# JohnGoertz/Gumbi

Hardware: AMD Instinct MI355X
Metric: fit+predict achieved GFLOP/s (fp64 exact GP: one MAP objective + gradient evaluation at the model's starting hyper-parameters + grid prediction) (higher is better)
Workload: dtype f64; 1 GPU; synthetic N=50k d=8 Matern-5/2 ARD fp64, M=10^4 grid; N=50000, d=8, kernel=Matern52, M=10000, parallelism=1 GPU, warmup_step=the same step (untimed)

## Files before the change

gumbi_amd/csrc/engine.hip:

```cpp
#include <hip/hip_runtime.h>

#include <algorithm>
#include <cmath>
#include <cstdarg>
#include <cstdio>
#include <cstdlib>
#include <cstring>
#include <string>
#include <functional>
#include <unordered_map>
#include <mutex>
#include <memory>
#include <vector>

#include "../../include/gumbi_hip.h"
#include "device_buffers.hpp"
#include "workspaces.hpp"
#include "term_walk.hpp"
#include "factor_state.hpp"
#include "eval_plan.hpp"
#include "covariance.hpp"
#include "gemm_f64.hpp"
#include "gemm_splitk.hpp"
#include "gradient.hpp"
// ... 84 lines not shown
  std::string err;

  int64_t N = 0, Np = 0, Nr = 0, ld = 0;
  int32_t D = 0;
  DevPool pool;
  DevBuf<double> dX, dy, dA;
  DevBuf<double> dDinv16;

  gmb_kernel_spec spec{};
  bool have_spec = false, have_theta = false;
  std::vector<double> theta;
  int nc_pad = 1;
  int periodic = 0;
  double periods[8] = {};
  PreparedPoints pts;
  DevBuf<double> dtabs, dnoise;
  struct Term {
    PrepArgs pa;
    CovParams cp;
    double eta;
    int n_tab_acc;
  };
  std::vector<Term> terms;
  std::vector<double> htabs;
  std::vector<double> hnoise;

  DevBuf<double> dscal;
  int32_t* dinfo = nullptr;
  DevBuf<double> dv;
  FactorState fs;
  DevBuf<double> dDiagSave;
  DevBuf<double> dsk;
  int64_t notpd = -1;
  double logdet = 0.0, vnorm2 = 0.0;

  PredictWorkspace pw;
  int predict_form = -1;
  GemmFormWorkspace pw2;
  JointState jt;
  DevBuf<double> dpart;
  PredictGradWorkspace pg;
  DevBuf<double> pg_part;
  DevBuf<double> dalpha_bs;
  DevBuf<double> vg_grad;
  TermsWorkspace tg;
  GroupWorkspace ga;
  DevBuf<double> ga_part;
  SlopeWorkspace slope;
  DevBuf<int64_t> ga_idx;
  DesignWorkspace dz;

  DevBuf<double> dW;
  DevBuf<double> dalpha;
  double* dgpart = nullptr;
  DevBuf<double> dgred;
  DevBuf<double> dgbig;

  struct InvLevelPlan {
    int variant[2] = {0, 0};
    int grid_x[2] = {0, 0};
    int count = 0;
    int64_t off[2] = {0, 0};
    int64_t toff = 0;
    int tr_rows = 0, tr_cols = 0;
    double flops[2] = {0.0, 0.0};
  };
  std::vector<InvLevelPlan> inv_plan;
  DevBuf<GemmArgs> dplan_gemm;
  DevBuf<TransposeJob> dplan_tr;
  int64_t plan_N = -1, plan_ld = -1, plan_Np = -1;
  const double* plan_W = nullptr;
  const double* plan_A = nullptr;
  bool batch_inverse = true;
  bool lpt_order = true;
  long long lpt_max_tiles = 16384;
  int cov_strip = 0;
  int tile_strip = 8;

  bool profiling = false;
  gmb_timings tm{};
  std::vector<EventPair> evs;
  bool naive_leaf = false;
  bool gemm_dma = true;
  bool small_tiles = true;
  int gemm_variant = 0;
  long long wg_slots = 512;
  bool force_variant = false;

  hipStream_t aux[3] = {nullptr, nullptr, nullptr};
  int chol_scheme = -1;
  DevBuf<uint32_t> dct;
  DevBuf<unsigned long long> dct_trace;
  bool ct_trace = false;
  CholResult chol;
  int ct_lose = 0;
  struct HostLanding {
    double scal[2];
    int32_t info;
    uint32_t abort;
    double gacc[GACC_DOUBLES];
  };
  HostLanding* hl = nullptr;
  HostLanding* hl_dev = nullptr;
  hipEvent_t fe[4] = {nullptr, nullptr, nullptr, nullptr};
  int inline_prep_max_rows = 4096;
  int grad_scheme = -1;
  int et_lag = -1;
  DevBuf<uint32_t> det_tasks;
  int et_key[5] = {-1, -1, -1, -1, -1};
  int et_pairs = -1;
  int et_pairs_min_blocks = 72;
  int et_ntasks = 0;
  DevBuf<double> dUdiag;
  DevBuf<double> dApart;
  int et_min_blocks = 1;
  int panel_tiles_w = 16;
  bool panel_tiles_veto = false;
  int tiles_min_blocks = 6, tiles_max_blocks = 224;
  int tiles_trsm_min_blocks = 16;
  int masked_max_blocks = 128;
  std::vector<hipEvent_t> sync_pool;
  size_t sync_next = 0;
  bool lookahead = true;
  bool par_inverse = true;
  bool aux_shared = false;
  bool aux_borrowed = false;
  int part_cus = 0;
  DevBuf<double> dsend, drecv;
  DevBuf<double> dsend2, drecv2;
  int panel_blocks = 8;
  bool panel_auto = true;
  int dist_mode = 0;
  DevBuf<double> dAown;
  int64_t ld_own = 0;
  int own_world = -1, own_rank = -1;
  DevBuf<double> dPanel;
  std::function<int(double*, int64_t, int)> solve_hook;
  DevBuf<double> dstat;
  uint64_t coll_count = 0, coll_hash = 0;
  std::vector<hipEvent_t> time_pool;
  size_t time_next = 0;
};

namespace {

int fail(gmb_engine* e, int code, const char* fmt, ...) {
  char buf[512];
  va_list ap;
  va_start(ap, fmt);
  vsnprintf(buf, sizeof buf, fmt, ap);
  va_end(ap);
  if (e) e->err = buf;
  return code;
}

#define HIP_TRY(e, call)                                                              \
  do {                                                                                \
    hipError_t _s = (call);                                                           \
    if (_s != hipSuccess)                                                             \
      return fail(e, GMB_EHIP, "%s failed: %s (%s:%d)", #call, hipGetErrorString(_s), \
                  __FILE__, __LINE__);                                                \
  } while (0)

int alloc_refused(void* owner, size_t bytes, const char* why) {
  return fail(static_cast<gmb_engine*>(owner), GMB_ENOMEM, "hipMalloc of %lld bytes failed: %s", (long long)bytes, why);
}
// ... 186 lines not shown
  if (g_in.mt <= 0 || g_in.nt <= 0 || g_in.k <= 0) return GMB_OK;
  GemmArgs g = g_in;
  if (g.nblk_stride < 1) g.nblk_stride = 1;
  const long long nact = gemm_nact128(g);
  const bool in_place = (const double*)g.C == g.B;
  int variant = e->gemm_variant;
  {
    static const double rate[4] = {73.0, 63.0, 65.0, 60.0};
    static const int per128[4] = {1, 4, 2, 4};
    const double slots = (double)e->wg_slots;
    auto score = [&](int v) {
      const double t = (double)(nact * per128[v]);
      const double rounds = std::max(1.0, t / slots + 0.5);
      return rate[v] * per128[v] / rounds;
    };
    if (in_place) {
      if (g.mt != 1) return fail(e, GMB_EINVAL, "internal: in-place GEMM needs m == 128");
      variant = 0;
      if (score(2) > score(variant)) variant = 2;
      if (score(3) > score(variant)) variant = 3;
      if (pin && pin->variant >= 0) {
        if (pin->variant != 0 && pin->variant != 2 && pin->variant != 3) return fail(e, GMB_EINVAL, "gemm pin: the in-place form runs on the 128-row tiles (variants 0, 2, 3)");
        variant = pin->variant;
      }
    } else if (pin && pin->variant >= 0) {
      if (pin->variant > 3) return fail(e, GMB_EINVAL, "gemm pin: variant %d", pin->variant);
      variant = pin->variant;
    } else if (!e->force_variant) {
      variant = 0;
      if (e->small_tiles) {
        if (score(2) > score(variant)) variant = 2;
        if (score(1) > score(variant)) variant = 1;
      }
    }
  }
#ifdef GMB_TUNING
  if (e->force_variant && e->gemm_variant == 4 && !in_place) variant = (g_in.mt % 2 == 0) ? 4 : 0;
#endif
  static const int BMs[5] = {128, 64, 128, 128, 256}, BNs[5] = {128, 64, 64, 32, 128};
  const int bm = BMs[variant], bn = BNs[variant];
  g.mt = g_in.mt * TILE / bm;
  g.nt = g_in.nt * TILE / bn;
  g.order = 0;
  if (e->lpt_order && nact <= e->lpt_max_tiles && g.nblk_stride == 1 && g.tri_off >= 0 && !g.klo_m && (g.klo_n != 0) != (g.khi_n != 0))
    g.order = g.klo_n ? 1 : 2;
  if (pin && pin->order >= 0) {
    const bool lpt_ok = g.nblk_stride == 1 && g.tri_off >= 0 && !g.klo_m && (g.klo_n != 0) != (g.khi_n != 0);
    if (pin->order > 2 || (pin->order != 0 && (!lpt_ok || pin->order != (g.klo_n ? 1 : 2))))
      return fail(e, GMB_EINVAL, "gemm pin: order %d is not one launch_gemm chooses for this product", pin->order);
    g.order = pin->order;
  }
  g.strip = (g.order == 0 && e->tile_strip > 0 && g.mt >= 2 && !in_place && !g.klo_m) ? e->tile_strip : 0;
  if (pin && pin->strip >= 0) {
    if (pin->strip > 255 || (pin->strip > 0 && !(g.order == 0 && g.mt >= 2 && !in_place && !g.klo_m)))
      return fail(e, GMB_EINVAL, "gemm pin: strip %d is not one launch_gemm chooses for this product", pin->strip);
    g.strip = pin->strip;
  }
  bool pfc = g.beta != 0.0 && g.k <= 1024 && !in_place;
  bool dma = e->gemm_dma && variant == 0 && !in_place;
  if (pin && pin->pfc >= 0) {
    if (pin->pfc > 1 || (pin->pfc == 1 && (g.beta == 0.0 || in_place || variant == 0)))
      return fail(e, GMB_EINVAL, "gemm pin: C prefetch needs beta != 0, an out-of-place product and a small tile");
    pfc = pin->pfc == 1;
  }
  if (pin && pin->staging >= 0) {
    if (pin->staging > 1 || (pin->staging == 1 && (variant != 0 || in_place)))
      return fail(e, GMB_EINVAL, "gemm pin: LDS-DMA staging exists for the out-of-place 128 x 128 tile only");
    dma = pin->staging == 1;
  }
  double flops = 0.0;
  const int nblocks = gemm_schedule(g, bm, bn, &flops);
  if (nblocks <= 0) return GMB_OK;
  const bool bulk_update = ev_kind == EV_CHOL_UPDATE && variant == 0 && !in_place;
  const int was_update = ev_kind == EV_CHOL_UPDATE ? (1 << 16) : 0;
  if (ev_kind == EV_CHOL_UPDATE && !bulk_update) ev_kind = EV_CHOL_PANEL_GEMM;
  ev_begin(e, s, ev_kind, flops, g_in.mt, g_in.nt, g.k,
           g.tri | (g.klo_n << 3) | (g.khi_n << 4) | (g.klo_m << 5) | (variant << 8) | was_update);
  const dim3 grid(nblocks);
  if (pin && pin->launched)
    *pin->launched = variant | (dma ? 4 : 0) | (variant != 0 && pfc ? 8 : 0) | (in_place ? 16 : 0) | (g.order << 5) | ((g.strip & 0xff) << 8) |
                     (std::min(nblocks, 0x7fff) << 16);
  switch (variant) {
    case 0:
      if (dma && bulk_update) hipLaunchKernelGGL(gemm_f64_dma_chol_update_kernel, grid, dim3(256), 0, s, g);
      else if (dma) hipLaunchKernelGGL(gemm_f64_dma_kernel, grid, dim3(256), 0, s, g);
      else hipLaunchKernelGGL((gemm_f64_kernel<2, 2, 4, 4, 2>), grid, dim3(256), 0, s, g);
      break;
#ifdef GMB_TUNING
    case 4: hipLaunchKernelGGL((gemm_f64_kernel<4, 2, 4, 4, 1>), grid, dim3(512), 0, s, g); break;
#endif
    case 1:
      if (pfc) hipLaunchKernelGGL((gemm_f64_kernel<2, 2, 2, 2, 2, true>), grid, dim3(256), 0, s, g);
      else hipLaunchKernelGGL((gemm_f64_kernel<2, 2, 2, 2, 2>), grid, dim3(256), 0, s, g);
      break;
    case 2:
      if (pfc) hipLaunchKernelGGL((gemm_f64_kernel<2, 2, 4, 2, 2, true>), grid, dim3(256), 0, s, g);
      else hipLaunchKernelGGL((gemm_f64_kernel<2, 2, 4, 2, 2>), grid, dim3(256), 0, s, g);
      break;
    default:
      if (pfc) hipLaunchKernelGGL((gemm_f64_kernel<2, 2, 4, 1, 2, true>), grid, dim3(256), 0, s, g);
      else hipLaunchKernelGGL((gemm_f64_kernel<2, 2, 4, 1, 2>), grid, dim3(256), 0, s, g);
      break;
  }
  ev_end(e);
  HIP_TRY(e, hipGetLastError());
  return GMB_OK;
}

int launch_trsm_strip(gmb_engine* e, hipStream_t s, double* B, int64_t ldb, int64_t nrows, const double* L, int64_t ldl,
                      const double* dinv16, int nvalid, EvKind ev_kind) {
  if (nrows <= 0) return GMB_OK;
  TrsmArgs t;
  t.B = B;
  t.ldb = ldb;
  t.nrows = nrows;
  t.L = L;
  t.ldl = ldl;
  t.dinv16 = dinv16;
  t.nvalid = nvalid;
  ev_begin(e, s, ev_kind, (double)nrows * TILE * TILE);
  hipLaunchKernelGGL(trsm_strip_kernel, dim3((unsigned)((nrows / 16 + 3) / 4)), dim3(256), 0, s, t);
  ev_end(e);
  HIP_TRY(e, hipGetLastError());
  return GMB_OK;
}

int launch_leaf(gmb_engine* e, hipStream_t s, const LeafArgs& a) {
  ev_begin(e, s, EV_LEAF, 0.0);
  if (e->naive_leaf)
    hipLaunchKernelGGL(potrf_leaf_naive_kernel, dim3(1), dim3(256), 0, s, a);
  else
    hipLaunchKernelGGL(potrf_leaf_kernel, dim3(1), dim3(512), 0, s, a);
  ev_end(e);
  HIP_TRY(e, hipGetLastError());
  return GMB_OK;
}

long long cov_grid_blocks(int ti, int tj, int strip, int tri_grid, int row_first, int row_stride) {
  const int S = strip < 1 ? 1 : strip;
  const long long nst = (tj + S - 1) / S;
  if (row_stride > 0) return row_first < ti ? ((ti - 1 - row_first) / row_stride + 1) * nst : 0;
  if (tri_grid) return cov_tri_blocks_before(ti, tj, S);
  return (long long)ti * nst;
}

template <int KIND>
int launch_cov_nc(gmb_engine* e, const CovTileArgs& a, int nc) {
  const long long nb = cov_grid_blocks(a.ti, a.tj, a.strip, a.tri_grid, a.row_first, a.row_stride) * (a.gsplit > 1 ? a.gsplit : 1);
  if (nb <= 0) return GMB_OK;
  const dim3 grid((unsigned)nb), block(256);
  switch (nc) {
    case 1: hipLaunchKernelGGL((cov_tile_kernel<KIND, 1>), grid, block, 0, e->stream, a); break;
    case 2: hipLaunchKernelGGL((cov_tile_kernel<KIND, 2>), grid, block, 0, e->stream, a); break;
    case 4: hipLaunchKernelGGL((cov_tile_kernel<KIND, 4>), grid, block, 0, e->stream, a); break;
    case 8: hipLaunchKernelGGL((cov_tile_kernel<KIND, 8>), grid, block, 0, e->stream, a); break;
    default: hipLaunchKernelGGL((cov_tile_kernel<KIND, 16>), grid, block, 0, e->stream, a); break;
  }
  HIP_TRY(e, hipGetLastError());
  return GMB_OK;
}

int launch_cov(gmb_engine* e, const CovTileArgs& a_in) {
  if (a_in.ti <= 0 || a_in.tj <= 0) return GMB_OK;
  CovTileArgs a = a_in;
  const double tiles = (double)a.ti * a.tj * (a.lower_only ? 0.5 : 1.0) / (a.row_stride > 0 ? a.row_stride : 1);
  a.stream_stores = tiles * TILE * TILE * 8.0 >= 1073741824.0 / (a.row_stride > 0 ? a.row_stride : 1);
  a.strip = e->cov_strip > 0 ? e->cov_strip : (tiles >= 32768.0 ? 4 : tiles >= 12288.0 ? 2 : 1);
// ... 1309 lines not shown
      }
    }
  if (k != (int)e->theta.size()) return fail(e, GMB_EINVAL, "internal: gradient packing mismatch");
  return GMB_OK;
}

inline bool chol_scheme_valid(int s) { return s == -1 || s == 0 || s == 2 || s == 3 || s == 4; }

int require_ready(gmb_engine* e, bool need_factor) {
  if (!e) return GMB_EINVAL;
  if (e->N <= 0) return fail(e, GMB_EINVAL, "gmb_set_data has not been called");
  if (!e->have_spec) return fail(e, GMB_EINVAL, "gmb_set_kernel has not been called");
  if (!e->have_theta) return fail(e, GMB_EINVAL, "gmb_set_theta has not been called");
  if (need_factor && !e->fs.valid())
    return fail(e, GMB_EINVAL, "no valid factorisation: call gmb_factorize first");
  return GMB_OK;
}

int require_full_factor(gmb_engine* e, const char* what) {
  if (e->fs.capacity() || !e->dA || e->dA.cap <= 0)
    return fail(e, GMB_EINVAL, "%s needs the complete factor on this device, but the resident factorisation is a capacity-mode one "
                               "(gmb_dist_set_mode(e, 1): no rank holds the factor) -- use the gmb_dist_* calls, or gmb_factorize first", what);
  return GMB_OK;
}

int require_capacity_factor(gmb_engine* e, const char* what) {
  if (!e->fs.capacity() || !e->dAown)
    return fail(e, GMB_EINVAL, "%s in capacity mode needs a factorisation made by gmb_dist_factorize in capacity mode; the resident "
                               "one was made by %s", what, e->fs.single() ? "gmb_factorize / gmb_evaluate" : "the replicated multi-GPU driver");
  return GMB_OK;
}

}

namespace {

hipStream_t shared_masked_stream(int device, int part_cus, int* ncu_out) {
  static std::mutex mu;
  static hipStream_t streams[64] = {};
  static int ncus[64] = {};
  std::lock_guard<std::mutex> lock(mu);
  hipStream_t& st = streams[device & 63];
  if (!st) {
    hipDeviceProp_t prop;
    if (hipGetDeviceProperties(&prop, device) != hipSuccess) return nullptr;
    const int ncu = prop.multiProcessorCount;
    std::vector<uint32_t> mask((ncu + 31) / 32, 0u);
    for (int i = part_cus; i < ncu; ++i) mask[i / 32] |= 1u << (i % 32);
    if (hipExtStreamCreateWithCUMask(&st, (uint32_t)mask.size(), mask.data()) != hipSuccess) {
      st = nullptr;
      (void)hipGetLastError();
      return nullptr;
    }
    ncus[device & 63] = ncu;
  }
  if (ncu_out) *ncu_out = ncus[device & 63];
  return st;
}

int gmb_create_impl(gmb_engine** out, int32_t device, void* stream, const gmb_engine* peer = nullptr) {
  if (!out) return GMB_EINVAL;
  *out = nullptr;
  int n = gmb_device_count();
  if (n < 0) return GMB_ENODEVICE;
  if (device < 0 || device >= n) return GMB_EINVAL;
  if (hipSetDevice(device) != hipSuccess) return GMB_EHIP;
  gmb_engine* e = new gmb_engine();
  e->device = device;
  if (stream) {
    e->stream = (hipStream_t)stream;
  } else {
    if (hipStreamCreateWithFlags(&e->stream, hipStreamNonBlocking) != hipSuccess) {
      delete e;
      return GMB_EHIP;
    }
    e->own_stream = true;
  }
  auto flag = [](const char* name, bool dflt) {
    const char* v = getenv(name);
    return v && v[0] ? v[0] != '0' : dflt;
  };
  e->naive_leaf = flag("GMB_LEAF_NAIVE", false);
  e->gemm_dma = flag("GMB_GEMM_DMA", true);
  const char* cs = getenv("GMB_CHOL_SCHEME");
  if (cs && cs[0]) {
    const int v = atoi(cs);
    if (chol_scheme_valid(v)) e->chol_scheme = v;
    else fprintf(stderr, "[gumbi_hip] GMB_CHOL_SCHEME=%s ignored: valid schemes are -1 (by size), 0, 2, 3, 4\n", cs);
  }
  int part = 32;
#ifdef GMB_TUNING
  e->small_tiles = flag("GMB_SMALL_TILES", true);
  const char* gv = getenv("GMB_GEMM_VARIANT");
  if (gv && gv[0] >= '0' && gv[0] <= '4') {
    e->gemm_variant = gv[0] - '0';
    e->force_variant = true;
  }
  e->lookahead = flag("GMB_LOOKAHEAD", true);
  e->lpt_order = flag("GMB_LPT_ORDER", true);
  if (const char* lm = getenv("GMB_LPT_MAX_TILES")) e->lpt_max_tiles = atoll(lm);
  const char* ts = getenv("GMB_TILE_STRIP");
  if (ts) e->tile_strip = std::max(0, atoi(ts));
  const char* cst = getenv("GMB_COV_STRIP");
  if (cst) e->cov_strip = std::max(0, std::min(64, atoi(cst)));
  e->batch_inverse = flag("GMB_BATCH_INVERSE", true);
  e->par_inverse = flag("GMB_PAR_INVERSE", true);
  const char* pb = getenv("GMB_PANEL_BLOCKS");
  if (pb && atoi(pb) > 0) {
    e->panel_blocks = atoi(pb);
    e->panel_auto = false;
  }
  const char* mb = getenv("GMB_MASKED_MAX_BLOCKS");
  if (mb) e->masked_max_blocks = atoi(mb);
  if (const char* pw = getenv("GMB_PANEL_TILES_W")) e->panel_tiles_w = std::max(0, std::min(64, atoi(pw)));
  const char* pc = getenv("GMB_PART_CUS");
  if (pc) part = atoi(pc);
#endif
  int prio_lo = 0, prio_hi = 0;
  (void)hipDeviceGetStreamPriorityRange(&prio_lo, &prio_hi);
  for (int a = 0; a < 3 && peer; ++a) {
    e->aux[a] = peer->aux[a];
    e->aux_borrowed = true;
    e->aux_shared = peer->aux_shared;
    e->part_cus = peer->part_cus;
  }
  for (int a = 0; a < 3 && !peer; ++a) {
    hipError_t st2 = hipSuccess;
    int ncu = 0;
    hipStream_t masked = (a == 2 && part > 0) ? shared_masked_stream(device, part, &ncu) : nullptr;
    if (masked) {
      e->aux[a] = masked;
      e->aux_shared = true;
      e->part_cus = part;
    } else {
      st2 = hipStreamCreateWithPriority(&e->aux[a], hipStreamNonBlocking, a == 2 ? prio_lo : prio_hi);
    }
    if (st2 != hipSuccess) {
      gmb_destroy(e);
      return GMB_EHIP;
    }
  }
  hipDeviceProp_t prop;
  if (hipGetDeviceProperties(&prop, device) == hipSuccess) e->wg_slots = 2LL * prop.multiProcessorCount;
  e->pool.owner = e;
  e->pool.refused = alloc_refused;
  if (e->dscal.renew(e->pool, SCAL_DOUBLES, false) || e->dstat.renew(e->pool, (DIST_HEADER + DIST_MAX_PAYLOAD) * (1 + DIST_MAX_WORLD), false)) {
    gmb_destroy(e);
    return GMB_ENOMEM;
  }
  e->dinfo = reinterpret_cast<int32_t*>(e->dscal + SCAL_INFO_AT);
  e->dgpart = e->dscal + SCAL_GACC_AT;
  *out = e;
  return GMB_OK;
}

}

extern "C" {

int gmb_abi_version(void) { return GMB_ABI_VERSION; }

int gmb_device_count(void) {
  int n = 0;
  hipError_t s = hipGetDeviceCount(&n);
  if (s != hipSuccess || n <= 0) return GMB_ENODEVICE;
  return n;
// ... 2577 lines not shown
  if (!out || ldo < e->Nr) return fail(e, GMB_EINVAL, "gmb_blk_covariance: out is null or ldo < %lld", (long long)e->Nr);
  if ((((uintptr_t)out) | (uintptr_t)(ldo * (int64_t)sizeof(double))) & 15u)
    return fail(e, GMB_EINVAL, "gmb_blk_covariance: out must be 16-byte aligned and ldo even (16-byte stores)");
  HIP_TRY(e, hipSetDevice(e->device));
  if ((rc = build_sigma(e, out, ldo))) return rc;
  HIP_TRY(e, hipStreamSynchronize(e->stream));
  return GMB_OK;
}

int gmb_blk_potrf(gmb_engine* e, double* Akk, int64_t lda, int32_t nvalid, double* dinv16,
                  double* logdet_accum, int32_t* info) {
  if (!e || !Akk || nvalid < 1 || nvalid > TILE || lda < TILE) return fail(e, GMB_EINVAL, "bad potrf block");
  HIP_TRY(e, hipSetDevice(e->device));
  LeafArgs a{};
  a.A = Akk;
  a.lda = lda;
  a.nvalid = nvalid;
  a.dinv16 = dinv16;
  a.logdet = logdet_accum;
  a.info = info ? info : e->dinfo;
  a.row0 = 0;
#ifdef GMB_TUNING
  a.dbg = getenv("GMB_LEAF_DBG") ? logdet_accum + 1 : nullptr;
#else
  a.dbg = nullptr;
#endif
  return launch_leaf(e, e->stream, a);
}

int gmb_blk_invert(gmb_engine* e, const double* Lkk, int64_t lda, int32_t nvalid, const double* dinv16,
                   double* invLkk) {
  if (!e || !Lkk || !dinv16 || !invLkk || nvalid < 1 || nvalid > TILE || lda < TILE)
    return fail(e, GMB_EINVAL, "bad invert block");
  HIP_TRY(e, hipSetDevice(e->device));
  InvArgs ia{};
  ia.L = Lkk;
  ia.lda = lda;
  ia.blk_stride = 0;
  ia.dinv16 = dinv16;
  ia.invL = invLkk;
  ia.n = nvalid;
  hipLaunchKernelGGL(leaf_invert_kernel, dim3(1), dim3(256), 0, e->stream, ia);
  HIP_TRY(e, hipGetLastError());
  return GMB_OK;
}

int gmb_blk_trsm(gmb_engine* e, double* B, int64_t ldb, int64_t nrows, const double* Lkk, int64_t ldl,
                 const double* dinv16, int32_t nvalid) {
  if (!e || !B || !Lkk || !dinv16 || nrows < 0 || nrows % 16 || ldb < nrows || ldl < TILE || nvalid < 1 ||
      nvalid > TILE)
    return fail(e, GMB_EINVAL, "bad trsm arguments (rows must be a multiple of 16)");
  HIP_TRY(e, hipSetDevice(e->device));
  return launch_trsm_strip(e, e->stream, B, ldb, nrows, Lkk, ldl, dinv16, nvalid, EV_CHOL_STRIP);
}

int gmb_blk_gemm_nt(gmb_engine* e, double* C, int64_t ldc, const double* A, int64_t lda, const double* B,
                    int64_t ldb, int64_t m, int64_t n, int64_t k, double alpha, double beta, int32_t tri,
                    int64_t tri_shift) {
  if (!e || !C || !A || !B) return fail(e, GMB_EINVAL, "null gemm operand");
  if (m % TILE || n % TILE || k % KT || m < 0 || n < 0 || k < 0)
    return fail(e, GMB_EINVAL, "gemm sizes must be multiples of 128 (m, n) and 16 (k)");
  HIP_TRY(e, hipSetDevice(e->device));
  GemmArgs g{};
  g.C = C;
  g.ldc = ldc;
  g.A = A;
  g.lda = lda;
  g.B = B;
  g.ldb = ldb;
  g.mt = (int)(m / TILE);
  g.nt = (int)(n / TILE);
  g.k = (int)k;
  g.alpha = alpha;
  g.beta = beta;
  g.tri = tri;
  g.tri_off = (int)(tri_shift * TILE);
  return launch_gemm(e, e->stream, g, EV_CHOL_PANEL_GEMM);
}

int gmb_blk_gemm_ex(gmb_engine* e, double* C, const double* A, const double* B, const gmb_gemm_desc* d, int32_t* launched) {
  if (launched) *launched = 0;
  if (!e) return GMB_EINVAL;
  if (!C || !A || !B || !d) return fail(e, GMB_EINVAL, "null gemm operand");
  if (d->m % TILE || d->n % TILE || d->k % KT || d->m < 0 || d->n < 0 || d->k < 0 || d->m > (1 << 24) || d->n > (1 << 24) || d->k > (1 << 24))
    return fail(e, GMB_EINVAL, "gemm sizes must be multiples of 128 (m, n) and 16 (k)");
  if (((uintptr_t)A | (uintptr_t)B | (uintptr_t)(d->lda * 8) | (uintptr_t)(d->ldb * 8)) & 15u)
    return fail(e, GMB_EINVAL, "gmb_blk_gemm_ex: A and B must be 16-byte aligned, lda and ldb even");
  if (d->nblk_stride < 0 || d->cblk_stride < 0 || d->krow_stride < 0 || d->nblk_stride > 4096 || d->cblk_stride > 4096 || d->krow_stride > 4096 ||
      (d->klo_m | d->klo_n | d->khi_n | d->tri) < 0 || (d->klo_m | d->klo_n | d->khi_n | d->tri) > 1)
    return fail(e, GMB_EINVAL, "gmb_blk_gemm_ex: strides must be >= 0, tri / klo_m / klo_n / khi_n 0 or 1");
  if (d->tri_off % 32 || d->krow_off % TILE) return fail(e, GMB_EINVAL, "gmb_blk_gemm_ex: tri_off must be a multiple of 32, krow_off of 128");
  const int64_t bs = d->nblk_stride < 1 ? 1 : d->nblk_stride, cs = d->cblk_stride > 0 ? d->cblk_stride : bs;
  const int64_t brows = d->n ? ((d->n / TILE - 1) * bs + 1) * TILE : 0, crows = d->n ? ((d->n / TILE - 1) * cs + 1) * TILE : 0;
  if (d->lda < d->m || d->ldb < brows || d->ldc < crows) return fail(e, GMB_EINVAL, "gmb_blk_gemm_ex: a leading dimension is smaller than its operand");
  if ((const double*)C == B && d->ldc != d->ldb) return fail(e, GMB_EINVAL, "gmb_blk_gemm_ex: in place needs ldc == ldb");
  if (d->variant < -1 || d->staging < -1 || d->pfc < -1 || d->order < -1 || d->strip < -1) return fail(e, GMB_EINVAL, "gmb_blk_gemm_ex: a pin below -1");
  HIP_TRY(e, hipSetDevice(e->device));
  GemmArgs g{};
  g.C = C;
  g.ldc = d->ldc;
  g.A = A;
  g.lda = d->lda;
  g.B = B;
  g.ldb = d->ldb;
  g.mt = (int)(d->m / TILE);
  g.nt = (int)(d->n / TILE);
  g.k = (int)d->k;
  g.alpha = d->alpha;
  g.beta = d->beta;
  g.tri = d->tri;
  g.tri_off = d->tri_off;
  g.nblk_stride = d->nblk_stride;
  g.cblk_stride = d->cblk_stride;
  g.klo_m = d->klo_m;
  g.klo_n = d->klo_n;
  g.khi_n = d->khi_n;
  g.krow_off = d->krow_off;
  g.krow_stride = d->krow_stride;
  GemmPin pin;
  pin.variant = d->variant;
  pin.staging = d->staging;
  pin.pfc = d->pfc;
  pin.order = d->order;
  pin.strip = d->strip;
  pin.launched = launched;
  return launch_gemm(e, e->stream, g, EV_CHOL_PANEL_GEMM, &pin);
}

int gmb_blk_gemm_splitk(gmb_engine* e, double* C, int64_t ldc, const double* A, int64_t lda, const double* B, int64_t ldb, int64_t m,
                        int64_t n, int64_t k, double alpha, double beta, int32_t tri, int32_t slices, int32_t* slices_used) {
  if (slices_used) *slices_used = 0;
  if (!e) return GMB_EINVAL;
  if (!C || !A || !B) return fail(e, GMB_EINVAL, "null gemm operand");
  if (m % TILE || n % TILE || k % KT || m <= 0 || n <= 0 || k <= 0 || m > (1 << 24) || n > (1 << 24) || k > (1 << 24))
    return fail(e, GMB_EINVAL, "split-k gemm sizes must be positive multiples of 128 (m, n) and 16 (k)");
  if (((uintptr_t)A | (uintptr_t)B | (uintptr_t)(lda * 8) | (uintptr_t)(ldb * 8)) & 15u)
    return fail(e, GMB_EINVAL, "gmb_blk_gemm_splitk: A and B must be 16-byte aligned, lda and ldb even");
  if (lda < m || ldb < n || ldc < n) return fail(e, GMB_EINVAL, "gmb_blk_gemm_splitk: a leading dimension is smaller than its operand");
  if (tri < 0 || tri > 1) return fail(e, GMB_EINVAL, "gmb_blk_gemm_splitk: tri must be 0 or 1");
  if (slices != -1 && slices < 1) return fail(e, GMB_EINVAL, "gmb_blk_gemm_splitk: slices must be -1 (by the rule) or >= 1");
  HIP_TRY(e, hipSetDevice(e->device));
  SplitKArgs a{};
  a.C = C;
  a.ldc = ldc;
  a.A = A;
  a.lda = lda;
  a.B = B;
  a.ldb = ldb;
  a.mt = (int)(m / TILE);
  a.nt = (int)(n / TILE);
  a.k = (int)k;
  a.alpha = alpha;
  a.beta = beta;
  a.tri = tri;
  return launch_gemm_splitk(e, e->stream, a, slices, slices_used);
}

int gmb_append(gmb_engine* e, const double* Xnew, int64_t K, int64_t ldx, const double* ynew, int32_t memspace) {
  int rc = resize_ready(e, "gmb_append");
  if (rc) return rc;
  if (!Xnew || !ynew || K < 0 || ldx < e->D) return fail(e, GMB_EINVAL, "gmb_append: bad Xnew/K/ldx/ynew");
  if (K == 0) return GMB_OK;
  return resize_n(e, e->N + K, Xnew, K, ldx, ynew, memspace, "gmb_append");
}

int64_t gmb_num_obs(const gmb_engine* e) { return e ? e->N : (int64_t)GMB_EINVAL; }

int gmb_truncate(gmb_engine* e, int64_t n_keep) {
// ... 52 lines not shown
```

gumbi_amd/csrc/gemm_f64.hpp:

```cpp
#pragma once
#include <hip/hip_runtime.h>
#include <algorithm>
#include <stdint.h>

namespace gmb {

typedef double d4 __attribute__((ext_vector_type(4)));
typedef double d2 __attribute__((ext_vector_type(2)));

constexpr int TILE = 128;
constexpr int KT = 16;
constexpr int PITCH = TILE + 16;

struct GemmArgs {
  double* C;
  int64_t ldc;
  const double* A;
  int64_t lda;
  const double* B;
  int64_t ldb;
  int32_t mt, nt;
  int32_t k;
  double alpha, beta;
  int32_t tri;
  int32_t tri_off;
  int32_t nblk_stride;
  int32_t cblk_stride;
  int32_t klo_m, klo_n, khi_n;
  int32_t krow_off;
  int32_t krow_stride;
  int32_t xstart[9];
  int32_t order;
  int32_t strip;
  int32_t xs_t0[8], xs_base[8];
};

__host__ __device__ __forceinline__ int xcd_remap(int bid, int nwg) {
  const int q = nwg >> 3, r = nwg & 7;
  const int xcd = bid & 7, idx = bid >> 3;
  const int base = (xcd < r) ? xcd * (q + 1) : r * (q + 1) + (xcd - r) * q;
  return base + idx;
}

__host__ __device__ __forceinline__ int64_t gemm_noff(int tn, int bn, int stride) {
  const int64_t e = (int64_t)tn * bn;
  return (e >> 7) * stride * 128 + (e & 127);
}
__host__ __device__ __forceinline__ int gemm_first_tn(int64_t T, int bn, int stride) {
  if (T <= 0) return 0;
  const int per = 128 / bn;
  if (T < 0x7fffffff) {
    const uint32_t S = (uint32_t)stride * 128u, t = (uint32_t)T;
    const uint32_t q = t / S, r = t - q * S;
    if (r == 0) return (int)(q * per);
    if (r > (uint32_t)(128 - bn)) return (int)((q + 1) * per);
    return (int)(q * per + (r + bn - 1) / (uint32_t)bn);
  }
  const int64_t S = (int64_t)stride * 128;
  const int64_t q = T / S, r = T % S;
  if (r == 0) return (int)(q * per);
  if (r > 128 - bn) return (int)((q + 1) * per);
  return (int)(q * per + (r + bn - 1) / bn);
}

__host__ __device__ inline bool gemm_decode_tile(const GemmArgs& g, const int BM, const int BN, const int vbid, int& tm,
                                                 int& tn) {
  const int xcd = vbid & 7;
  int ci = g.xstart[xcd] + (vbid >> 3);
  if (g.order == 0 && g.strip > 0) {
    if (ci >= g.xstart[xcd + 1]) return false;
    auto first_of = [&](int t) {
      if (!g.tri) return 0;
      const int f = gemm_first_tn((int64_t)t * BM - g.tri_off - (BN - 1), BN, g.nblk_stride);
      return f > g.nt ? g.nt : f;
    };
    int t0 = g.xs_t0[xcd];
    ci -= g.xs_base[xcd];
    for (;;) {
      const int t1 = t0 + g.strip < g.mt ? t0 + g.strip : g.mt;
      int cnt = 0;
      for (int t = t0; t < t1; ++t) cnt += g.nt - first_of(t);
      if (ci < cnt) break;
      ci -= cnt;
      t0 = t1;
      if (t0 >= g.mt) return false;
    }
// ... 124 lines not shown
#pragma unroll
    for (int p = 0; p < NA; ++p) *reinterpret_cast<d2*>(&As[(a_row + RA * p) * PA + a_col]) = ra[p];
#pragma unroll
    for (int p = 0; p < NB; ++p) *reinterpret_cast<d2*>(&Bs[(b_row + RB * p) * PB + b_col]) = rb[p];
  };

  auto compute = [&](int st) {
    const double* As = &lds[st][0];
    const double* Bs = &lds[st][KT * PA];
#pragma unroll
    for (int k4 = 0; k4 < KT; k4 += 4) {
      double a[WTM], b[WTN];
#pragma unroll
      for (int i = 0; i < WTM; ++i) a[i] = As[(k4 + kq) * PA + wm * (16 * WTM) + i * 16 + r16];
#pragma unroll
      for (int j = 0; j < WTN; ++j) b[j] = Bs[(k4 + kq) * PB + wn * (16 * WTN) + j * 16 + r16];
#pragma unroll
      for (int i = 0; i < WTM; ++i)
#pragma unroll
        for (int j = 0; j < WTN; ++j)
          acc[i][j] = __builtin_amdgcn_mfma_f64_16x16x4f64(a[i], b[j], acc[i][j], 0, 0, 0);
    }
  };

  if (kt0 < kt1) {
    gload(kt0);
    lstore(0);
    __syncthreads();
    int st = 0;
    constexpr int NMFMA = WTM * WTN * (KT / 4), NMEM = NA + NB;
    constexpr int SLOT = NMFMA / (4 * NMEM) > 0 ? NMFMA / (4 * NMEM) : 1;
    static_assert(2 * SLOT * NMEM <= NMFMA, "not enough MFMAs to interleave the staging with");
    for (int kt = kt0; kt + 1 < kt1; ++kt) {
      gload(kt + 1);
      compute(st);
      lstore(st ^ 1);
#pragma unroll
      for (int q = 0; q < NMEM; ++q) {
        __builtin_amdgcn_sched_group_barrier(0x008, SLOT, 0);
        __builtin_amdgcn_sched_group_barrier(0x020, 1, 0);
      }
      __builtin_amdgcn_sched_group_barrier(0x008, NMFMA - 2 * SLOT * NMEM, 0);
#pragma unroll
      for (int q = 0; q < NMEM; ++q) {
        __builtin_amdgcn_sched_group_barrier(0x008, SLOT, 0);
        __builtin_amdgcn_sched_group_barrier(0x200, 1, 0);
      }
      __syncthreads();
      st ^= 1;
    }
    compute(st);
  }


  double* __restrict__ Cg = g.C + (g.cblk_stride > 0 ? gemm_noff(tn, BN, g.cblk_stride) : noff) + wn * (16 * WTN) + r16;
  const int64_t m0 = (int64_t)tm * BM + wm * (16 * WTM) + kq;
  if (g.beta == 0.0) {
#pragma unroll
    for (int i = 0; i < WTM; ++i)
#pragma unroll
      for (int r = 0; r < 4; ++r) {
        double* row = Cg + (m0 + i * 16 + 4 * r) * g.ldc;
#pragma unroll
        for (int j = 0; j < WTN; ++j) row[j * 16] = g.alpha * acc[i][j][r];
      }
  } else {
#pragma unroll
    for (int i = 0; i < WTM; ++i)
#pragma unroll
      for (int r = 0; r < 4; ++r) {
        double* row = Cg + (m0 + i * 16 + 4 * r) * g.ldc;
        double c[WTN];
#pragma unroll
        for (int j = 0; j < WTN; ++j) {
          if constexpr (PREFETCH_C) c[j] = prefetch_c ? cpre[(i * 4 + r) * WTN + j] : row[j * 16];
          else c[j] = row[j * 16];
        }
#pragma unroll
        for (int j = 0; j < WTN; ++j) row[j * 16] = g.beta * c[j] + g.alpha * acc[i][j][r];
      }
  }
}

template <bool DUMMY = false>
__device__ __forceinline__ void gemm_f64_dma_body(const GemmArgs& g, const int vbid) {
  constexpr int WGN = 2, WTM = 4, WTN = 4;
  constexpr int BM = 128, BN = 128, PA = BM + 16, PB = BN + 16;
  constexpr int KD = 8, NS = 4;
  constexpr int STAGE = KD * (PA + PB);
  typedef __attribute__((address_space(3))) double lds_double;
  typedef __attribute__((address_space(3))) void lds_void;
  typedef const __attribute__((address_space(1))) void g_void;
  __shared__ __attribute__((aligned(16))) double lds_[NS * STAGE];
  lds_double* const lds = (lds_double*)lds_;

  int tm, tn;
  if (!gemm_decode_tile(g, BM, BN, vbid, tm, tn)) return;
  const int tid = threadIdx.x;
  const int lane = tid & 63;
  const int wave = __builtin_amdgcn_readfirstlane(tid >> 6);
  const int wm = wave / WGN, wn = wave % WGN;
  const int r16 = lane & 15, kq = lane >> 4;

  const int krow = (int)gemm_noff(tn, BN, g.krow_stride > 0 ? g.krow_stride : g.nblk_stride) + g.krow_off;
  int k_lo = g.klo_m * tm * BM + g.klo_n * krow;
  int k_hi = g.k;
  if (g.khi_n) k_hi = min(k_hi, krow + BN);
  if (k_lo < 0) k_lo = 0;
  if (k_lo > k_hi) k_lo = k_hi;
  const int64_t noff = gemm_noff(tn, BN, g.nblk_stride);
  const int kt0 = k_lo / KD, kt1 = k_hi / KD;

  d4 acc[WTM][WTN];
#pragma unroll
  for (int i = 0; i < WTM; ++i)
#pragma unroll
    for (int j = 0; j < WTN; ++j) acc[i][j] = d4{0.0, 0.0, 0.0, 0.0};

  const double* pa = g.A + (int64_t)tm * BM + ((int64_t)kt0 * KD + wave) * g.lda;
  const double* pb = g.B + noff + ((int64_t)kt0 * KD + wave) * g.ldb;
  const int lane2 = 2 * lane;
  int issued = kt0;
  auto dma = [&](const int stage) {
    lds_double* As = lds + stage * STAGE + wave * PA;
    lds_double* Bs = lds + stage * STAGE + KD * PA + wave * PB;
    __builtin_amdgcn_global_load_lds((g_void*)(pa + lane2), (lds_void*)As, 16, 0, 0);
    __builtin_amdgcn_global_load_lds((g_void*)(pb + lane2), (lds_void*)Bs, 16, 0, 0);
    __builtin_amdgcn_global_load_lds((g_void*)(pa + 4 * g.lda + lane2), (lds_void*)(As + 4 * PA), 16, 0, 0);
    __builtin_amdgcn_global_load_lds((g_void*)(pb + 4 * g.ldb + lane2), (lds_void*)(Bs + 4 * PB), 16, 0, 0);
    if (issued + 1 < kt1) {
      pa += (int64_t)KD * g.lda;
      pb += (int64_t)KD * g.ldb;
      ++issued;
    }
  };
  double fa[2][WTM], fb[2][WTN];
  auto frags = [&](const int kt, const int k4, const int buf) {
    const lds_double* As = lds + (kt & (NS - 1)) * STAGE + (4 * k4 + kq) * PA + r16;
    const lds_double* Bs = lds + (kt & (NS - 1)) * STAGE + KD * PA + (4 * k4 + kq) * PB + r16;
#pragma unroll
    for (int i = 0; i < WTM; ++i) fa[buf][i] = As[wm * (16 * WTM) + i * 16];
#pragma unroll
    for (int j = 0; j < WTN; ++j) fb[buf][j] = Bs[wn * (16 * WTN) + j * 16];
  };
  auto mfmas = [&](const int buf) {
#pragma unroll
    for (int i = 0; i < WTM; ++i)
#pragma unroll
      for (int j = 0; j < WTN; ++j) acc[i][j] = __builtin_amdgcn_mfma_f64_16x16x4f64(fa[buf][i], fb[buf][j], acc[i][j], 0, 0, 0);
  };
  auto pin_step = [&]() {
#pragma unroll
    for (int q = 0; q < 4; ++q) {
      __builtin_amdgcn_sched_group_barrier(0x008, 2, 0);
      __builtin_amdgcn_sched_group_barrier(0x100, 1, 0);
    }
    __builtin_amdgcn_sched_group_barrier(0x008, WTM * WTN - 8, 0);
  };

  if (kt0 < kt1) {
    dma(kt0 & (NS - 1));
    dma((kt0 + 1) & (NS - 1));
    dma((kt0 + 2) & (NS - 1));
    dma((kt0 + 3) & (NS - 1));
    asm volatile("s_waitcnt vmcnt(12)" ::: "memory");
    __builtin_amdgcn_s_barrier();
    frags(kt0, 0, 0);
    for (int kt = kt0; kt < kt1; ++kt) {
      frags(kt, 1, 1);
      mfmas(0);
      pin_step();
      asm volatile("s_waitcnt vmcnt(8) lgkmcnt(0)" ::: "memory");
      __builtin_amdgcn_s_barrier();
      dma(kt & (NS - 1));
      frags(kt + 1, 0, 0);
      mfmas(1);
      pin_step();
    }
    asm volatile("s_waitcnt vmcnt(0)" ::: "memory");
  }

  double* __restrict__ Cg = g.C + (g.cblk_stride > 0 ? gemm_noff(tn, BN, g.cblk_stride) : noff) + wn * (16 * WTN) + r16;
  const int64_t m0 = (int64_t)tm * BM + wm * (16 * WTM) + kq;
  if (g.beta == 0.0) {
#pragma unroll
    for (int i = 0; i < WTM; ++i)
#pragma unroll
      for (int r = 0; r < 4; ++r) {
        double* row = Cg + (m0 + i * 16 + 4 * r) * g.ldc;
#pragma unroll
        for (int j = 0; j < WTN; ++j) row[j * 16] = g.alpha * acc[i][j][r];
      }
  } else {
#pragma unroll
    for (int i = 0; i < WTM; ++i)
#pragma unroll
      for (int r = 0; r < 4; ++r) {
        double* row = Cg + (m0 + i * 16 + 4 * r) * g.ldc;
        double c[WTN];
#pragma unroll
        for (int j = 0; j < WTN; ++j) c[j] = row[j * 16];
#pragma unroll
        for (int j = 0; j < WTN; ++j) row[j * 16] = g.beta * c[j] + g.alpha * acc[i][j][r];
      }
  }
}

__global__ __launch_bounds__(256, 2) void gemm_f64_dma_kernel(GemmArgs g) {
  gemm_f64_dma_body<>(g, blockIdx.x);
}

__global__ __launch_bounds__(256, 2) void gemm_f64_dma_chol_update_kernel(GemmArgs g) {
  gemm_f64_dma_body<>(g, blockIdx.x);
}

template <int WGM, int WGN, int WTM, int WTN, int OCC, bool PFC = false>
__global__ __launch_bounds__(64 * WGM * WGN, OCC) void gemm_f64_kernel(GemmArgs g) {
  gemm_f64_body<WGM, WGN, WTM, WTN, PFC>(g, blockIdx.x);
}

template <int WGM, int WGN, int WTM, int WTN, int OCC>
__global__ __launch_bounds__(64 * WGM * WGN, OCC) void gemm_f64_batched_kernel(const GemmArgs* __restrict__ batch) {
  const GemmArgs g = batch[blockIdx.y];
  gemm_f64_body<WGM, WGN, WTM, WTN>(g, blockIdx.x);
}

__global__ __launch_bounds__(256, 2) void mfma_f64_peak_kernel(double* sink, int iters, double scale) {
  d4 acc[4][4];
#pragma unroll
  for (int i = 0; i < 4; ++i)
#pragma unroll
    for (int j = 0; j < 4; ++j) acc[i][j] = d4{0.0, 0.0, 0.0, 0.0};
  double a[4], b[4];
#pragma unroll
  for (int i = 0; i < 4; ++i) {
    a[i] = scale * (1.0 + 1e-9 * (threadIdx.x + i));
    b[i] = scale * (1.0 - 1e-9 * (threadIdx.x + 7 * i));
  }
  const long long t0 = __builtin_readcyclecounter();
  for (int it = 0; it < iters; ++it) {
#pragma unroll
    for (int i = 0; i < 4; ++i)
#pragma unroll
      for (int j = 0; j < 4; ++j)
        acc[i][j] = __builtin_amdgcn_mfma_f64_16x16x4f64(a[i], b[j], acc[i][j], 0, 0, 0);
  }
  double s = 0.0;
#pragma unroll
  for (int i = 0; i < 4; ++i)
#pragma unroll
    for (int j = 0; j < 4; ++j) s += acc[i][j][0] + acc[i][j][1] + acc[i][j][2] + acc[i][j][3];
  const long long t1 = __builtin_readcyclecounter();
  if (s == 12345.678) sink[0] = s;
  if (blockIdx.x == 0 && threadIdx.x == 0) sink[1] = (double)(t1 - t0);
}

inline int gemm_schedule(GemmArgs& g, int bm, int bn, double* flops) {
  const int KU = g.k / KT;
  auto first_of = [&](int tm) {
    if (!g.tri) return 0;
    const int f = gemm_first_tn((int64_t)tm * bm - g.tri_off - (bn - 1), bn, g.nblk_stride);
    return f > g.nt ? g.nt : f;
  };
  auto kunits = [&](int tm, int tn) {
    const int kstride = g.krow_stride > 0 ? g.krow_stride : (g.nblk_stride < 1 ? 1 : g.nblk_stride);
    const int krow = (int)gemm_noff(tn, bn, kstride) + g.krow_off;
    const int lo = std::max(0, g.klo_m * tm * bm + g.klo_n * krow) / KT;
    int hi = KU;
    if (g.khi_n && (krow + bn) / KT < hi) hi = (krow + bn) / KT;
    return hi > lo ? hi - lo : 0;
  };
  if (g.order != 0) {
    long long nact = 0, funits = 0;
    for (int tn = 0; tn < g.nt; ++tn) {
      long long cnt = g.mt;
      if (g.tri) cnt = std::min<long long>(cnt, ((long long)tn * bn + bn - 1 + g.tri_off) / bm + 1);
      nact += cnt;
      funits += cnt * kunits(0, tn);
    }
    if (flops) *flops = 2.0 * bm * bn * KT * (double)funits;
    for (int i = 0; i <= 8; ++i) g.xstart[i] = 0;
    return (int)nact;
  }
  static thread_local long long* P = nullptr;
  static thread_local long long* F = nullptr;
  static thread_local int cap = 0;
  if (cap < g.nt + 1) {
    delete[] P;
    delete[] F;
    cap = g.nt + 1;
    P = new long long[cap];
    F = new long long[cap];
  }
  const int fixed = 4;
  P[0] = F[0] = 0;
  for (int tn = 0; tn < g.nt; ++tn) {
// ... 89 lines not shown
```

Before: 70000 GFLOP/s.

## Peel DMA GEMM tail to drain pipeline and prefetch C during last tiles

Splits the LDS-DMA GEMM main loop so the final NS k-tiles run in a peeled tail. The tail uses progressively tighter waitcnts instead of one full vmcnt(0) drain and, when beta is nonzero, interleaves loads of the C tile with the final MFMAs so the beta*C epilogue is overlapped with compute. This targets the exposed epilogue and drain latency in the Cholesky trailing update and other accumulating GEMMs. It adds register pressure from the prefetched C values, hand-tuned vmcnt counts that must match the DMA issue pattern, and an env flag that falls back to the old plain kernels.

```diff
diff --git a/gumbi_amd/csrc/engine.hip b/gumbi_amd/csrc/engine.hip
--- a/gumbi_amd/csrc/engine.hip
+++ b/gumbi_amd/csrc/engine.hip
@@ -190,6 +190,7 @@
   std::vector<EventPair> evs;
   bool naive_leaf = false;
   bool gemm_dma = true;
+  bool gemm_seams = true;
   bool small_tiles = true;
   int gemm_variant = 0;
   long long wg_slots = 512;
@@ -542,7 +543,10 @@
                      (std::min(nblocks, 0x7fff) << 16);
   switch (variant) {
     case 0:
-      if (dma && bulk_update) hipLaunchKernelGGL(gemm_f64_dma_chol_update_kernel, grid, dim3(256), 0, s, g);
+      if (dma && !e->gemm_seams && bulk_update) hipLaunchKernelGGL(gemm_f64_dma_chol_update_plain_kernel, grid, dim3(256), 0, s, g);
+      else if (dma && !e->gemm_seams) hipLaunchKernelGGL(gemm_f64_dma_plain_kernel, grid, dim3(256), 0, s, g);
+      else if (dma && bulk_update && g.beta != 0.0) hipLaunchKernelGGL(gemm_f64_dma_chol_update_kernel, grid, dim3(256), 0, s, g);
+      else if (dma && g.beta != 0.0) hipLaunchKernelGGL(gemm_f64_dma_acc_kernel, grid, dim3(256), 0, s, g);
       else if (dma) hipLaunchKernelGGL(gemm_f64_dma_kernel, grid, dim3(256), 0, s, g);
       else hipLaunchKernelGGL((gemm_f64_kernel<2, 2, 4, 4, 2>), grid, dim3(256), 0, s, g);
       break;
@@ -2018,6 +2022,7 @@
   };
   e->naive_leaf = flag("GMB_LEAF_NAIVE", false);
   e->gemm_dma = flag("GMB_GEMM_DMA", true);
+  e->gemm_seams = flag("GMB_GEMM_SEAMS", true);
   const char* cs = getenv("GMB_CHOL_SCHEME");
   if (cs && cs[0]) {
     const int v = atoi(cs);
@@ -4761,8 +4766,9 @@
   if (launched) *launched = 0;
   if (!e) return GMB_EINVAL;
   if (!C || !A || !B || !d) return fail(e, GMB_EINVAL, "null gemm operand");
-  if (d->m % TILE || d->n % TILE || d->k % KT || d->m < 0 || d->n < 0 || d->k < 0 || d->m > (1 << 24) || d->n > (1 << 24) || d->k > (1 << 24))
-    return fail(e, GMB_EINVAL, "gemm sizes must be multiples of 128 (m, n) and 16 (k)");
+  const int kq = (d->variant == 0 && d->staging == 1) ? 8 : KT;
+  if (d->m % TILE || d->n % TILE || d->k % kq || d->m < 0 || d->n < 0 || d->k < 0 || d->m > (1 << 24) || d->n > (1 << 24) || d->k > (1 << 24))
+    return fail(e, GMB_EINVAL, "gemm sizes must be multiples of 128 (m, n) and 16 (k; 8 when pinned to the LDS-DMA kernel)");
   if (((uintptr_t)A | (uintptr_t)B | (uintptr_t)(d->lda * 8) | (uintptr_t)(d->ldb * 8)) & 15u)
     return fail(e, GMB_EINVAL, "gmb_blk_gemm_ex: A and B must be 16-byte aligned, lda and ldb even");
   if (d->nblk_stride < 0 || d->cblk_stride < 0 || d->krow_stride < 0 || d->nblk_stride > 4096 || d->cblk_stride > 4096 || d->krow_stride > 4096 ||
diff --git a/gumbi_amd/csrc/gemm_f64.hpp b/gumbi_amd/csrc/gemm_f64.hpp
--- a/gumbi_amd/csrc/gemm_f64.hpp
+++ b/gumbi_amd/csrc/gemm_f64.hpp
@@ -2,6 +2,7 @@
 #include <hip/hip_runtime.h>
 #include <algorithm>
 #include <stdint.h>
+#include <type_traits>
 
 namespace gmb {
 
@@ -292,7 +293,7 @@
   }
 }
 
-template <bool DUMMY = false>
+template <int SEAMS = 0, bool BNZ = false>
 __device__ __forceinline__ void gemm_f64_dma_body(const GemmArgs& g, const int vbid) {
   constexpr int WGN = 2, WTM = 4, WTN = 4;
   constexpr int BM = 128, BN = 128, PA = BM + 16, PB = BN + 16;
@@ -368,7 +369,84 @@
     __builtin_amdgcn_sched_group_barrier(0x008, WTM * WTN - 8, 0);
   };
 
-  if (kt0 < kt1) {
+  auto plain_epilogue = [&]() {
+    double* __restrict__ Cg = g.C + (g.cblk_stride > 0 ? gemm_noff(tn, BN, g.cblk_stride) : noff) + wn * (16 * WTN) + r16;
+    const int64_t m0 = (int64_t)tm * BM + wm * (16 * WTM) + kq;
+    if (g.beta == 0.0) {
+#pragma unroll
+      for (int i = 0; i < WTM; ++i)
+#pragma unroll
+        for (int r = 0; r < 4; ++r) {
+          double* row = Cg + (m0 + i * 16 + 4 * r) * g.ldc;
+#pragma unroll
+          for (int j = 0; j < WTN; ++j) row[j * 16] = g.alpha * acc[i][j][r];
+        }
+    } else {
+#pragma unroll
+      for (int i = 0; i < WTM; ++i)
+#pragma unroll
+        for (int r = 0; r < 4; ++r) {
+          double* row = Cg + (m0 + i * 16 + 4 * r) * g.ldc;
+          double c[WTN];
+#pragma unroll
+          for (int j = 0; j < WTN; ++j) c[j] = row[j * 16];
+#pragma unroll
+          for (int j = 0; j < WTN; ++j) row[j * 16] = g.beta * c[j] + g.alpha * acc[i][j][r];
+        }
+    }
+  };
+
+  if constexpr (SEAMS == 0) {
+    if (kt0 < kt1) {
+      dma(kt0 & (NS - 1));
+      dma((kt0 + 1) & (NS - 1));
+      dma((kt0 + 2) & (NS - 1));
+      dma((kt0 + 3) & (NS - 1));
+      asm volatile("s_waitcnt vmcnt(12)" ::: "memory");
+      __builtin_amdgcn_s_barrier();
+      frags(kt0, 0, 0);
+      for (int kt = kt0; kt < kt1; ++kt) {
+        frags(kt, 1, 1);
+        mfmas(0);
+        pin_step();
+        asm volatile("s_waitcnt vmcnt(8) lgkmcnt(0)" ::: "memory");
+        __builtin_amdgcn_s_barrier();
+        dma(kt & (NS - 1));
+        frags(kt + 1, 0, 0);
+        mfmas(1);
+        pin_step();
+      }
+      asm volatile("s_waitcnt vmcnt(0)" ::: "memory");
+    }
+  } else {
+    auto pin_step_c = [&]() {
+#pragma unroll
+      for (int q = 0; q < 4; ++q) {
+        __builtin_amdgcn_sched_group_barrier(0x008, 1, 0);
+        __builtin_amdgcn_sched_group_barrier(0x020, 1, 0);
+        __builtin_amdgcn_sched_group_barrier(0x008, 1, 0);
+        __builtin_amdgcn_sched_group_barrier(0x020, 1, 0);
+        __builtin_amdgcn_sched_group_barrier(0x100, 1, 0);
+      }
+#pragma unroll
+      for (int q = 0; q < 8; ++q) {
+        __builtin_amdgcn_sched_group_barrier(0x008, 1, 0);
+        __builtin_amdgcn_sched_group_barrier(0x020, 1, 0);
+      }
+    };
+    double* __restrict__ Cg = g.C + (g.cblk_stride > 0 ? gemm_noff(tn, BN, g.cblk_stride) : noff) + wn * (16 * WTN) + r16;
+    const int64_t m0 = (int64_t)tm * BM + wm * (16 * WTM) + kq;
+    double cpre[2][BNZ ? 4 * WTN : 1];
+    auto cload = [&](const int i, const int b) {
+#pragma unroll
+      for (int r = 0; r < 4; ++r)
+#pragma unroll
+        for (int j = 0; j < WTN; ++j) cpre[b][r * WTN + j] = Cg[(m0 + i * 16 + 4 * r) * g.ldc + j * 16];
+    };
+    if (kt0 >= kt1) {
+      plain_epilogue();
+      return;
+    }
     dma(kt0 & (NS - 1));
     dma((kt0 + 1) & (NS - 1));
     dma((kt0 + 2) & (NS - 1));
@@ -376,7 +454,8 @@
     asm volatile("s_waitcnt vmcnt(12)" ::: "memory");
     __builtin_amdgcn_s_barrier();
     frags(kt0, 0, 0);
-    for (int kt = kt0; kt < kt1; ++kt) {
+    int kt = kt0;
+    for (; kt < kt1 - NS; ++kt) {
       frags(kt, 1, 1);
       mfmas(0);
       pin_step();
@@ -387,41 +466,85 @@
       mfmas(1);
       pin_step();
     }
-    asm volatile("s_waitcnt vmcnt(0)" ::: "memory");
-  }
-
-  double* __restrict__ Cg = g.C + (g.cblk_stride > 0 ? gemm_noff(tn, BN, g.cblk_stride) : noff) + wn * (16 * WTN) + r16;
-  const int64_t m0 = (int64_t)tm * BM + wm * (16 * WTM) + kq;
-  if (g.beta == 0.0) {
-#pragma unroll
-    for (int i = 0; i < WTM; ++i)
-#pragma unroll
-      for (int r = 0; r < 4; ++r) {
-        double* row = Cg + (m0 + i * 16 + 4 * r) * g.ldc;
-#pragma unroll
-        for (int j = 0; j < WTN; ++j) row[j * 16] = g.alpha * acc[i][j][r];
-      }
-  } else {
-#pragma unroll
-    for (int i = 0; i < WTM; ++i)
-#pragma unroll
-      for (int r = 0; r < 4; ++r) {
-        double* row = Cg + (m0 + i * 16 + 4 * r) * g.ldc;
-        double c[WTN];
-#pragma unroll
-        for (int j = 0; j < WTN; ++j) c[j] = row[j * 16];
-#pragma unroll
-        for (int j = 0; j < WTN; ++j) row[j * 16] = g.beta * c[j] + g.alpha * acc[i][j][r];
-      }
-  }
+    auto tail = [&](auto pf) {
+      constexpr bool PF = decltype(pf)::value;
+      auto tile = [&](auto tt) {
+        constexpr int T = decltype(tt)::value;
+        frags(kt, 1, 1);
+        mfmas(0);
+        pin_step();
+        if constexpr (T == 0) asm volatile("s_waitcnt vmcnt(8) lgkmcnt(0)" ::: "memory");
+        else if constexpr (T == 1 && PF) asm volatile("s_waitcnt vmcnt(20) lgkmcnt(0)" ::: "memory");
+        else if constexpr (T == 1) asm volatile("s_waitcnt vmcnt(4) lgkmcnt(0)" ::: "memory");
+        else if constexpr (T == 2 && PF) asm volatile("s_waitcnt vmcnt(32) lgkmcnt(0)" ::: "memory");
+        else if constexpr (T == 2) asm volatile("s_waitcnt vmcnt(0) lgkmcnt(0)" ::: "memory");
+        else asm volatile("s_waitcnt lgkmcnt(0)" ::: "memory");
+        if constexpr (T < NS - 1) {
+          __builtin_amdgcn_s_barrier();
+          if constexpr (PF && T < 2) cload(T, T);
+          frags(kt + 1, 0, 0);
+        }
+        mfmas(1);
+        if constexpr (PF && T < 2) pin_step_c();
+        else if constexpr (T < NS - 1) pin_step();
+      };
+      tile(std::integral_constant<int, 0>{});
+      if (++kt < kt1) {
+        tile(std::integral_constant<int, 1>{});
+        if (++kt < kt1) {
+          tile(std::integral_constant<int, 2>{});
+          if (++kt < kt1) tile(std::integral_constant<int, 3>{});
+        }
+      }
+    };
+    if constexpr (!BNZ) tail(std::false_type{});
+    if constexpr (!BNZ) asm volatile("s_waitcnt vmcnt(0)" ::: "memory");
+    if constexpr (BNZ) {
+      {
+        tail(std::true_type{});
+        if (kt1 - kt0 < 2) cload(1, 1);
+        __builtin_amdgcn_s_waitcnt(0x0F70);
+#pragma unroll
+        for (int i = 0; i < WTM; ++i) {
+          double out[4 * WTN];
+#pragma unroll
+          for (int r = 0; r < 4; ++r)
+#pragma unroll
+            for (int j = 0; j < WTN; ++j) out[r * WTN + j] = g.beta * cpre[i & 1][r * WTN + j] + g.alpha * acc[i][j][r];
+          __builtin_amdgcn_sched_barrier(0);
+          if (i + 2 < WTM) cload(i + 2, i & 1);
+          __builtin_amdgcn_sched_barrier(0);
+#pragma unroll
+          for (int r = 0; r < 4; ++r) {
+            double* row = Cg + (m0 + i * 16 + 4 * r) * g.ldc;
+#pragma unroll
+            for (int j = 0; j < WTN; ++j) row[j * 16] = out[r * WTN + j];
+          }
+          __builtin_amdgcn_sched_barrier(0);
+        }
+        return;
+      }
+    }
+  }
+
+  plain_epilogue();
 }
 
 __global__ __launch_bounds__(256, 2) void gemm_f64_dma_kernel(GemmArgs g) {
-  gemm_f64_dma_body<>(g, blockIdx.x);
+  gemm_f64_dma_body<1, false>(g, blockIdx.x);
+}
+__global__ __launch_bounds__(256, 2) void gemm_f64_dma_acc_kernel(GemmArgs g) {
+  gemm_f64_dma_body<1, true>(g, blockIdx.x);
+}
+__global__ __launch_bounds__(256, 2) void gemm_f64_dma_plain_kernel(GemmArgs g) {
+  gemm_f64_dma_body<0>(g, blockIdx.x);
 }
 
 __global__ __launch_bounds__(256, 2) void gemm_f64_dma_chol_update_kernel(GemmArgs g) {
-  gemm_f64_dma_body<>(g, blockIdx.x);
+  gemm_f64_dma_body<1, true>(g, blockIdx.x);
+}
+__global__ __launch_bounds__(256, 2) void gemm_f64_dma_chol_update_plain_kernel(GemmArgs g) {
+  gemm_f64_dma_body<0>(g, blockIdx.x);
 }
 
 template <int WGM, int WGN, int WTM, int WTN, int OCC, bool PFC = false>
```

Result: no change. 69990 GFLOP/s, median of 2 (-0.0%).
